# kngwyu/rogue-gym

Measured on AMD Instinct MI355X. Metric: env-steps/sec (whole node) at 65 536 envs, 32x16 mini-dungeon, higher is better.
Workload: dtype u8/u16 integer state, f32 observation; 1 GPU; config-mini.json 32x16, 65536 envs per GPU (65536 total), gray-image obs [N,1,16,32] f32, max_steps 1000, auto-reset; envs_per_gpu=65536, parallelism=env-sharded x1, no data-path collective

## Files before the change

### rogue-gym_amd/csrc/rg_api.cpp

```cpp
#include <hip/hip_runtime.h>
#include <dlfcn.h>

#include <algorithm>
#include <cstdio>
#include <cstdlib>
#include <cstring>
#include <mutex>
#include <random>
#include <string>
#include <vector>

#include "../../include/rogue_gym_hip.h"
#include "rg_state.h"
#include "rg_state_io.h"
#include "rg_action_mask.h"
#include "rg_path.h"
#include "rg_route.h"
#include "rg_episode.h"
#include "rg_monsters.h"

extern "C" {
typedef struct ncclComm *ncclComm_t;
typedef struct { char internal[128]; } ncclUniqueId;
typedef int ncclResult_t;
// ... 11 lines not shown
void rgk_export(const RgState *S, uint32_t *err_any, void *o_screen, void *o_hist, void *o_status, void *o_flags, uint32_t *o_err, hipStream_t st);
int rgk_regen_lanes_supported(const RgConfig *c, int maze_cap);
int rgk_step_bound_capable(const RgConfig *c);
int rgk_regen_lanes(const RgState *SP, const RgConfig *c, uint32_t *q, int32_t *list, int bulk, int waves, int slots, hipStream_t st, hipEvent_t ev0, hipEvent_t ev1);
void rgk_debug_descend(const RgState *S, const RgConfig *c, hipStream_t st);
void rgk_render(const RgState *S, const RgConfig *c, hipStream_t st);
void rgk_encode(const uint8_t *screen, const uint8_t *hist, const int32_t *status, uint32_t *flags, uint32_t *err_any, int n, int hw, size_t rs, size_t rst,
                int symbols, int planes_sym, uint32_t sflag, int with_hist, int kind, float *out, const int32_t *ext, hipStream_t st);
void rgk_pack(const RgState *S, int with_hist, uint8_t *out, hipStream_t st);
void rgk_scatter_rows(const void *src, void *dst, const int32_t *ext, int n, int row_bytes, hipStream_t st);
void rgk_gather_keys(const uint8_t *keys, const int32_t *ext, uint8_t *dst, int n, hipStream_t st);
int rgk_obs(const RgState *S, const RgConfig *c, uint32_t sflag, int with_hist, int kind, float *out, uint32_t *err_any, int planes_sym, int bound, hipStream_t st, hipEvent_t ev0, hipEvent_t ev1);
int rgk_redraw(const RgState *S, const RgConfig *c, hipStream_t st);
int rgk_obs_tail_capable(const RgState *S, const RgConfig *c);
int rgk_step_tail_capable(const RgConfig *c);
void rgk_obs_resid(const RgState *S, const RgConfig *c, float *out, hipStream_t st, hipEvent_t ev0, hipEvent_t ev1);
int rgk_obs_typed(const RgState *S, const RgConfig *c, int kind, int dtype, uint32_t sflag, int with_hist, int planes_sym, void *out, uint32_t *err_any, hipStream_t st, hipEvent_t ev0,
                  hipEvent_t ev1);
int rgk_obs_crop(const RgState *S, const RgConfig *c, int kind, int ry, int rx, uint32_t sflag, int with_hist, int planes_sym, float *out, int32_t *centers,
                 uint32_t *err_any, hipStream_t st);
int rgk_crop_typed(const RgState *S, const RgConfig *c, int kind, int dtype, int ry, int rx, uint32_t sflag, int with_hist, int planes_sym, void *out, int32_t *centers,
                   uint32_t *err_any, hipStream_t st, hipEvent_t ev0, hipEvent_t ev1);
void rgk_action_mask(const RgState *S, const RgConfig *c, const uint8_t *keys, int n_keys, uint8_t *mask, uint8_t *sample, uint64_t seed, uint64_t draw, hipStream_t st,
                     hipEvent_t ev0, hipEvent_t ev1);
void rgk_path(const RgState *S, const RgConfig *c, uint32_t goals, const int32_t *gcell, uint16_t *field, int32_t *dist, uint8_t *key, hipStream_t st);
void rgk_route(const RgState *S, const RgConfig *c, uint32_t goals, uint32_t fallback, uint32_t mode, const int32_t *gcell, int32_t *dist, uint8_t *key, uint8_t *tier,
               hipStream_t st);
void rgk_episode(const RgState *S, const RgConfig *c, const RgEpisode *A, int slots, const int32_t *ids, const uint8_t *mask, int cut, int record, uint32_t serial,
                 hipStream_t st);
void rgk_monsters(const RgState *S, const RgConfig *c, uint32_t mode, int cap, int16_t *table, int32_t *threat, hipStream_t st);
void rgk_state_save(const RgState *S, const RgIoLayout *L, const uint64_t *desc, const uint32_t *guard, const int32_t *ids, int k, uint8_t *out, hipStream_t st);
void rgk_state_load(const RgState *S, const RgIoLayout *L, const uint64_t *desc, const uint32_t *guard, const int32_t *ids, int k, const uint8_t *recs, uint32_t rec_bytes, uint8_t *ok,
                    uint8_t *mark, hipStream_t st);
void rgk_state_stairs(const RgState *S, const RgIoLayout *L, uint8_t *mark, hipStream_t st);
void rgk_reset_compact(const uint8_t *mask, int n, int32_t *list, uint32_t *cnt, hipStream_t st);
void rgk_build_list(const RgState *S, const RgConfig *c, const int32_t *list, const uint32_t *cnt, uint8_t *mark, hipStream_t st);
}

#define RG_ENC_CUT_TICKS 4000u
#define RG_TIMED_KERNELS 5
struct rg_handle {
    RgParsed parsed;
    RgConfig cfg;
    RgState S;
    RgState SP;
    bool spares = false;
    uint32_t *lane_q = nullptr; int32_t *lane_list = nullptr;
    hipStream_t side3 = nullptr;
    hipStream_t side2 = nullptr;
    int lane_flip = 0;
    uint64_t lane_last = 0;
    uint8_t *pin_keys = nullptr;
    uint32_t *pin_err = nullptr;
    bool lane_regen = false;
    uint64_t step_count = 0;
    hipStream_t side = nullptr;
    int regen_idle_after = -1;
    int regen_bulk = 0;
    int device = 0;
    hipStream_t stream = nullptr;
    std::vector<void *> allocs;
    uint32_t *d_err = nullptr;
    uint8_t *d_keys = nullptr;
    bool render_pending = false;
    float *bound_out = nullptr; int bound_kind = 0; bool bound_valid = false;
    int32_t *obs_list_mem = nullptr; uint32_t *obs_cnt_mem = nullptr; float *gray_lut_mem = nullptr;
    bool tail_enc = false, tail_enc_off = false;
    int bound_steps = 0;
    int stair_gen = 0;
    float *obs_scratch = nullptr;
    size_t obs_scratch_cap = 0;
    std::vector<uint64_t> seed_lo, seed_hi;
    std::vector<uint8_t> reseed;
    std::vector<uint64_t> range_lo, range_span;
    unsigned long long *d_probe = nullptr;
    std::vector<rg_handle *> sub;
    std::vector<int> g_of, l_of;
    int32_t *d_ext = nullptr;
    std::vector<int32_t> ext;
    uint8_t *d_keys_sub = nullptr;
    int planes_sym = 0;
    bool screens_stale = true;
// ... 160 lines not shown
              dev_alloc(h, &S.dlevel, n) && dev_alloc(h, &S.steps, n) && dev_alloc(h, &S.flags, n) && dev_alloc(h, &S.reward, n) && dev_alloc(h, &S.done, n) &&
              dev_alloc(h, &S.rng, 12 * n) && dev_alloc(h, &S.seed_lo, n) && dev_alloc(h, &S.seed_hi, n) && dev_alloc(h, &S.reseed, n) &&
              dev_alloc(h, &S.room_rect, nr * n) && dev_alloc(h, &S.room_meta, nr * n) &&
              dev_alloc(h, &S.mon_w0, nr * n) && dev_alloc(h, &S.mon_hp, nr * n) && dev_alloc(h, &S.mon_exp, nr * n) &&
              dev_alloc(h, &S.mon_cnt, n) && dev_alloc(h, &S.gold_pos, nr * n) && dev_alloc(h, &S.gold_amt, nr * n) &&
              dev_alloc(h, &S.edge_a, ne * n) && dev_alloc(h, &S.edge_b, ne * n) &&
              dev_alloc(h, &S.maze_stack, (size_t)maze_cap * n) && dev_alloc(h, &S.build_ctr, n) && dev_alloc(h, &S.stats, RG_STAT_COLS * h->stat_rows) && dev_alloc(h, &S.stair_list, 2 * n) && dev_alloc(h, &S.stair_cnt, 8) && dev_alloc(h, &S.stair_mark, 2 * n) &&
              dev_alloc(h, &S.dc_map, h->cfg.n_enemies > 0 ? n * RG_DIST_SLOTS * hw : 16) && dev_alloc(h, &S.dc_key, RG_DIST_SLOTS * n) &&
              dev_alloc(h, &S.dc_head, n) && dev_alloc(h, &S.dc_len, n) && dev_alloc(h, &S.dc_part, n) && dev_alloc(h, &S.dc_own, n) && dev_alloc(h, &S.status, n * 10) &&
              dev_alloc(h, &h->d_err, 4) && dev_alloc(h, &h->d_keys, n);
    if (ok && nr <= RG_OBS_MAX_ROOMS) ok = dev_alloc(h, &S.obs_rec, n * (size_t)RG_OBS_REC_WORDS(nr));
    if (ok && nr <= RG_OVL_MAX && getenv("ROGUE_GYM_HIP_NO_MIRROR_UPDATE") == nullptr)
        ok = dev_alloc(h, &S.ovl, (nr + 1) * n) && hipMemset(S.ovl, 0xff, (nr + 1) * n * 2) == hipSuccess;
    {
        if (ok && rgk_step_tail_capable(&h->cfg) && S.ovl && S.obs_rec) {
            ok = dev_alloc(h, &S.enc_stamp, n) && ensure_gray_lut(h) == 0;
            h->tail_enc = ok;
            S.enc_cut = RG_ENC_CUT_TICKS;
            if (const char *ev = RG_DEV_ENV("ROGUE_GYM_HIP_ENC_CUT")) S.enc_cut = (uint32_t)atoi(ev);
        }
    }
    h->spares = auto_reset != 0 && getenv("ROGUE_GYM_HIP_NO_SPARES") == nullptr;
    h->lane_regen = h->spares && getenv("ROGUE_GYM_HIP_WAVE_REGEN") == nullptr && rgk_regen_lanes_supported(&h->cfg, maze_cap) > 0;
    const char *slots_env = getenv("ROGUE_GYM_HIP_SP_SLOTS");
    S.sp_slots = h->lane_regen ? (slots_env ? atoi(slots_env) : 4) : 1;
    if (S.sp_slots < 1 || S.sp_slots > 8) S.sp_slots = 4;
    const size_t ns = n * (size_t)S.sp_slots;
    ok = ok && dev_alloc(h, &S.sp_ready, ns) && dev_alloc(h, &h->d_probe, 4) && dev_alloc(h, &S.launch_mark, 4);
    if (ok && h->cfg.n_enemies > 0 && RG_PARTIAL_MAPS(h->cfg.width, h->cfg.height, (int)nr))
        ok = dev_alloc(h, &S.dc_walk, n * RG_DIST_SLOTS * h->cfg.height * RG_WALK_WORDS(h->cfg.width));
    S.full_bfs = getenv("ROGUE_GYM_HIP_FULL_BFS") != nullptr;
    S.keep_spares = getenv("ROGUE_GYM_HIP_KEEP_SPARES") != nullptr;
    S.err_any = h->d_err;
    if (ok && !h->range_lo.empty()) {
// ... 251 lines not shown
    }
    h->S.stair_gen = h->stair_gen++;
    { TimedLaunch t(h, 3); rgk_build(&h->S, &h->cfg, h->stream); }
    HIPCHK(h, hipGetLastError());
    h->render_pending = true;
    h->bound_valid = false;
    return 0;
}

static int obs_common(rg_t *h, uint32_t status_flag, int with_hist, int kind, float *out_dev);
int rg_step(rg_t *h, const uint8_t *keys, int keys_on_device) { return rg_step_prefix(h, keys, h->S.n, keys_on_device); }
int rg_step_obs_gray(rg_t *h, const uint8_t *keys, int keys_on_device, uint32_t status_flag, int with_hist, float *out_dev) {
    const bool enc = h->tail_enc && !h->tail_enc_off && h->sub.empty() && (status_flag & 0x1ffu) == 0 && !with_hist && !h->bound_out && out_dev && rgk_obs_tail_capable(&h->S, &h->cfg);
    if (enc) {
        h->S.enc_out = out_dev;
        h->S.enc_step = (uint32_t)(h->step_count % 0xffffffffull) + 1u;
    }
    const int rc = rg_step_prefix(h, keys, h->S.n, keys_on_device);
    h->S.enc_out = nullptr;
    if (rc) return 1;
    if (!enc) return obs_common(h, status_flag, with_hist, 0, out_dev);
    {
        TimedLaunch t(h, 2, true);
        rgk_obs_resid(&h->S, &h->cfg, out_dev, h->stream, t.start_ev(), t.stop_ev());
    }
    HIPCHK(h, hipGetLastError());
    h->render_pending = false;
    h->bound_valid = false;
    h->bound_steps = 0;
    return 0;
}

int rg_step_prefix(rg_t *h, const uint8_t *keys, int n_keys, int keys_on_device) {
    HIPCHK(h, hipSetDevice(h->device));
// ... 1491 lines not shown
```

### rogue-gym_amd/csrc/rg_kernels.hip

```cpp


#include "rg_device.h"


#include "rg_gen.h"


#ifdef RG_FINE_PROF
#define PFM(id) pf.mark(id)
#else
#define PFM(id) ((void)0)
#endif
struct Prof {
    unsigned long long *p; unsigned long long t, t0, r0; int k;
    __device__ __forceinline__ void start(unsigned long long *pp) { p = pp ? pp + (size_t)blockIdx.x * 64 : nullptr; k = 0; if (p) { r0 = __builtin_amdgcn_s_memrealtime(); t = t0 = __builtin_amdgcn_s_memtime(); } }
    __device__ __forceinline__ void rec(int phase, unsigned long long v) {
        if (p && threadIdx.x == 0 && k < 61) p[1 + k++] = ((unsigned long long)phase << 48) | (v & 0xffffffffffffull);
    }
    __device__ __forceinline__ void mark(int phase) {
        if (!p) return;
        unsigned long long now = __builtin_amdgcn_s_memtime();
        rec(phase, now - t);
        t = now;
    }
// ... 2036 lines not shown
    }
    if (did_hit) react |= R_STATUS;
    return false;
}

__device__ __forceinline__ uint32_t base_glyph(const RgConfig &c, uint32_t v, int y) {
    const bool inner = y >= 1 && y < c.height - 1;
    uint32_t gl = ' ';
    if (inner && (v & C_VISIBLE)) gl = glyph_of(v);
    if (inner && (v & (C_VISIBLE | C_DRAWN))) gl = ((v & C_GOLD) ? (uint32_t)'*' : gl) | 0x80u;
    return gl;
}
#define OVL_SHOW 0x80u
#define OVL_UNKNOWN 0x40u
#define OVL_NONE 0xffffu
template <bool BND>
__device__ __forceinline__ bool mirror_update(const RgState &S, const RgConfig &c, const Env &E, const Win &w, uint32_t react, int rid0) {
    const int W = c.width, nrooms = c.room_num_x * c.room_num_y, n = E.n;
    int e = E.e;
    asm volatile("" : "+v"(e));
    uint8_t *scr = S.screen + (size_t)e * S.hw;
    float *og = (BND && S.bound_gray) ? S.bound_gray + (size_t)e * S.hw : nullptr;
    const __attribute__((address_space(3))) float *lutg = (const __attribute__((address_space(3))) float *)(g_smem + STEP_LDS_LUT);
    auto put = [&](int idx, uint32_t g) {
        scr[idx] = (uint8_t)g;
        if constexpr (BND) { if (og) og[idx] = lutg[g & 0x7fu]; }
    };
    int ln = threadIdx.x;
    asm volatile("" : "+v"(ln));
    const lds_u32 *mc = (const lds_u32 *)(g_smem + STEP_LDS_MC) + ln;
    const lds_u32 *ovl_l = (const lds_u32 *)(g_smem + STEP_LDS_OVL) + ln;
    const uint32_t ds = ovl_l[0] & 0x1ffffffu;
    const int px = E.px, py = E.py, rid = room_id_of(c, px, py);
    auto in_win = [&](int x, int y) { const int i = x - w.ox, j = y - w.oy; return i >= -2 && i <= 2 && j >= -2 && j <= 2; };
    auto dirty_at = [&](int x, int y) { return in_win(x, y) && ((ds >> WIN_K(x - w.ox, y - w.oy)) & 1u); };
    const int rsel = rid == rid0 ? 0 : 2;
    const uint32_t r_rect = ovl_l[(RG_OVL_MAX + 2 + rsel) * WAVE], r_meta = ovl_l[(RG_OVL_MAX + 3 + rsel) * WAVE] & 0xffu;
    const __attribute__((address_space(3))) uint8_t *mt = (const __attribute__((address_space(3))) uint8_t *)(ovl_l - ln + (RG_OVL_MAX + 6) * WAVE);
    uint32_t actp = 0;
    bool far = false;
// ... 135 lines not shown
                if (s0 + k < nrooms) {
                    const size_t g = (size_t)(s0 + k) * n + e;
                    S.room_rect[g] = rr[k]; S.room_meta[g] = rm[k]; S.mon_w0[g] = mw[k]; S.mon_hp[g] = mh[k]; S.mon_exp[g] = me[k]; S.gold_pos[g] = gp[k]; S.gold_amt[g] = ga[k];
                    if (S.obs_rec) {
                        uint32_t *rec = S.obs_rec + (size_t)e * RG_OBS_REC_WORDS(nrooms);
                        rec[s0 + k] = mw[k]; rec[nrooms + 1 + s0 + k] = rr[k]; reinterpret_cast<uint8_t *>(&rec[2 * nrooms + 1])[s0 + k] = rm[k];
                    }
                    if (S.ovl) S.ovl[(size_t)(s0 + k) * n + e] = (uint16_t)(((mw[k] >> 24) & MF_ALIVE) ? ((mw[k] & 0xffffu) | 0x40u) : 0xffffu);
                }
        }
    }
    __syncthreads();
    if (taken && !(S.keep_spares && S.reseed[e] == 0)) __hip_atomic_store(&S.sp_ready[es], 0u, __ATOMIC_RELAXED, __HIP_MEMORY_SCOPE_AGENT);
}

#ifndef ENC_BATCH
#define ENC_BATCH 8
#endif
__device__ __forceinline__ void tail_encode(const RgState &S, const int lane, const int e, const bool encl) {
    typedef float f4v __attribute__((ext_vector_type(4)));
    const uint64_t em = __ballot(encl);
    if (encl) S.enc_stamp[e] = S.enc_step;
    if (!em) return;
    const int ebase = __builtin_amdgcn_readfirstlane(e - lane);
    asm volatile("s_waitcnt vmcnt(0)" ::: "memory");
    const __attribute__((address_space(3))) float *lut = (const __attribute__((address_space(3))) float *)(g_smem + STEP_LDS_LUT);
    const uint32_t *mir = reinterpret_cast<const uint32_t *>(S.screen) + lane;
    f4v *img = reinterpret_cast<f4v *>(S.enc_out) + lane;
    uint64_t rem = em;
    int last = 0;
    struct Batch { int env[ENC_BATCH]; uint32_t w0[ENC_BATCH], w1[ENC_BATCH]; };
    auto load = [&](Batch &b) {
#pragma unroll
        for (int k = 0; k < ENC_BATCH; k++) {
            last = rem ? __builtin_ctzll(rem) : last;
            rem &= rem - (rem ? 1ull : 0ull);
            b.env[k] = ebase + last;
            const uint32_t *m = mir + (size_t)b.env[k] * 128;
            b.w0[k] = __hip_atomic_load(m, __ATOMIC_RELAXED, __HIP_MEMORY_SCOPE_AGENT);
            b.w1[k] = __hip_atomic_load(m + WAVE, __ATOMIC_RELAXED, __HIP_MEMORY_SCOPE_AGENT);
        }
    };
    auto gray4 = [&](uint32_t w) {
        w &= 0x7f7f7f7fu;
        f4v v = {lut[w & 0xff], lut[(w >> 8) & 0xff], lut[(w >> 16) & 0xff], lut[w >> 24]};
        return v;
    };
    auto store = [&](const Batch &b) {
#pragma unroll
        for (int k = 0; k < ENC_BATCH; k++) {
            f4v *o = img + (size_t)b.env[k] * 128;
            __builtin_nontemporal_store(gray4(b.w0[k]), o);
            __builtin_nontemporal_store(gray4(b.w1[k]), o + WAVE);
        }
    };
    const int nb = (__popcll(em) + ENC_BATCH - 1) / ENC_BATCH;
    Batch cur, nxt;
    load(cur);
    load(nxt);
    store(cur);
#pragma nounroll
    for (int b = 1; b < nb; b++) {
        cur = nxt;
        load(nxt);
        store(cur);
    }
}

template <int BW, int GM, bool BND = false, bool ENC = false>
__device__ __forceinline__ void step_wave(const RgState &S, const RgState *__restrict__ SPd, const RgConfig &c, const uint8_t *__restrict__ keys, int use_spares, int stage_off,
                                          const int e, const bool valid_in, const int stair_role) {
    uint16_t *lds_grid = reinterpret_cast<uint16_t *>(g_smem + stage_off);
    const int lane = threadIdx.x;
    Prof pf; pf.start(S.prof);
    const unsigned long long enc_t0 = ENC ? __builtin_amdgcn_s_memrealtime() : 0ull;
    Env E;
    E.err = 0; E.on_stairs = 0;
    uint32_t react = 0, err = 0, old_flags = 0, steps = 0, flags = 0;
    int act = ACT_NOOP, dir = 0;
    int gold0 = 0;
    bool live = false;
    bool ui_dead = false, terminal = false;
    bool inc_done = false;
    bool taken = false;
    uint32_t n_bfs = 0, n_inline = 0, n_taken = 0, n_cont = 0;
    uint32_t key = 0, nxs = RG_NX_NONE;
    bool listed = false;
    const int nrooms_k = c.room_num_x * c.room_num_y;
    E.mc = (lds_u32 *)(g_smem + STEP_LDS_MC) + lane;
    const uint32_t glyph_r = S.ovl ? c.mon[lane & 31].tile : 0u;
    if (valid_in) {
        listed = S.stair_mark[(size_t)(S.stair_gen & 1) * S.n + e] != 0;
        uint32_t nxk = 0;
        if (S.nx_state) {
            nxs = __hip_atomic_load(&S.nx_state[e], __ATOMIC_RELAXED, __HIP_MEMORY_SCOPE_AGENT);
            nxk = __hip_atomic_load(&S.nx_rng[(size_t)3 * S.n + e], __ATOMIC_RELAXED, __HIP_MEMORY_SCOPE_AGENT);
        }
        old_flags = S.flags[e];
// ... 19 lines not shown
            act = decode_key(key, dir);
            if (act == ACT_INVALID) err = RG_FLAG_ERR_KEY;
            else {
                klog_push(S, e, key);
                if (old_flags & RG_FLAG_DEAD) err = RG_FLAG_ERR_DEAD;
                else live = true;
            }
        }
    }
    pf.mark(0);
    bool need_gen = false, descends = false;
    Win w;
    w.v = (lds_u16 *)(g_smem + STEP_LDS_WIN) + lane;
    lds_u32 *ovl_l = (lds_u32 *)(g_smem + STEP_LDS_OVL) + lane;
    ovl_l[0] = 0;
    if ((BND && S.bound_gray) || ENC) {
        typedef const __attribute__((address_space(1))) void *gptr;
        typedef __attribute__((address_space(3))) void *lptr;
        __builtin_amdgcn_global_load_lds((gptr)(S.gray_lut + lane), (lptr)(g_smem + STEP_LDS_LUT), 4, 0, 0);
        __builtin_amdgcn_global_load_lds((gptr)(S.gray_lut + 64 + lane), (lptr)(g_smem + STEP_LDS_LUT + 256), 4, 0, 0);
    }
    if (S.ovl && lane < RG_MAX_ENEMY_KINDS + 6)
        ((__attribute__((address_space(3))) uint8_t *)(g_smem + STEP_LDS_OVL + (RG_OVL_MAX + 6) * WAVE * 4))[lane] = (uint8_t)glyph_r;
    if (S.ovl) {
        typedef const __attribute__((address_space(1))) void *gptr;
        typedef __attribute__((address_space(3))) void *lptr;
        lds_u32 *base = (lds_u32 *)(g_smem + STEP_LDS_OVL);
        const size_t es = valid_in ? (size_t)e : 0;
#pragma unroll
        for (int s0 = 0; s0 <= RG_OVL_MAX; s0++)
            __builtin_amdgcn_global_load_lds((gptr)(S.ovl + (size_t)(s0 <= nrooms_k ? s0 : 0) * S.n + es), (lptr)(base + (1 + s0) * WAVE), 2, 0, 0);
// ... 138 lines not shown
            if (running) win_load(c, E.cell, w, E.px, E.py);
        }
        if (live) {
            flags = (react & 0x7f00u);
            if (react & R_REDRAW) flags |= RG_FLAG_REDRAW | ((react & R_HIST_STALE) ? RG_FLAG_HIST_STALE : 0);
            else flags |= old_flags & (RG_FLAG_REDRAW | RG_FLAG_HIST_STALE);
            flags |= old_flags & (RG_FLAG_HIST_LAG | RG_FLAG_HIST_DIRTY | (BND ? RG_FLAG_SCR_CHANGED : 0u));
            if ((react & R_HIST_CHANGED) || descends) flags |= RG_FLAG_HIST_DIRTY;
            if (react & R_STATUS) write_status(S, c, E);
            if (ui_dead) flags |= RG_FLAG_DEAD;
            steps += 1;
            terminal = (react & R_GRAVE) || steps >= c.max_steps;
            need_gen = terminal && c.auto_reset;
            if (S.ovl && (react & R_REDRAW) && !descends && !need_gen && act != ACT_MOVE_UNTIL &&
                !(old_flags & (RG_FLAG_REDRAW | RG_FLAG_HIST_STALE | RG_FLAG_HIST_LAG | RG_FLAG_HIST_DIRTY)) && !(ovl_l[0] >> 31)) {
                if (mirror_update<BND>(S, c, E, w, react, room_id_of(c, w.ox, w.oy))) flags = (flags & ~(RG_FLAG_REDRAW | RG_FLAG_HIST_DIRTY)) | ((!BND || S.bound_gray) ? 0u : RG_FLAG_SCR_CHANGED);
                inc_done = true;
            }
        }
    }
    pf.mark(6);
    int et = e;
    asm volatile("" : "+v"(et));
    E.e = et;
    bool pend = false; uint64_t pm = 0; uint32_t lbase = 0;
    bool encl = false;
    if (BND && S.obs_list) {
        const uint32_t fw = (live ? ((terminal && c.auto_reset) ? RG_FLAG_REDRAW : flags) : old_flags);
        pend = valid && (fw & (RG_FLAG_REDRAW | RG_FLAG_SCR_CHANGED));
        pm = __ballot(pend);
        if (pm && lane == 0) lbase = atomicAdd(&S.obs_cnt[S.obs_par], (uint32_t)__popcll(pm));
    }
    if (S.stats) {
        const uint32_t cnt[8] = {(uint32_t)__popcll(__ballot(live && terminal && c.auto_reset)), (uint32_t)__popcll(__ballot(descends)),
                                 wave_sum(n_bfs), wave_sum(n_inline), wave_sum(n_taken), (uint32_t)__popcll(__ballot(live && (react & R_REDRAW))),
                                 (uint32_t)__popcll(__ballot(live)), (BW == 1 || BW == 2) ? wave_sum(n_cont) : 0u};
        const uint32_t n_nx = (uint32_t)__popcll(__ballot(descends && nxs == RG_NX_HIT));
        int ln = threadIdx.x;
        asm volatile("" : "+v"(ln));
        if (ln < RG_STAT_COLS) {
            uint32_t mine = ln == 8 ? n_nx : 0u;
// ... 13 lines not shown
        if (terminal && c.auto_reset) {
            if (taken) {
                E.dlevel = 1; E.gold = c.init_gold; E.hp = E.hpmax = c.init_hp; E.plvl = 1; E.exp = 0; E.food = c.hunger_time;
            }
            write_status(S, c, E);
            S.dc_len[et] = 0; S.dc_head[et] = 0; S.dc_part[et] = 0; S.dc_own[et] = 0;
            steps = 0;
            flags = RG_FLAG_REDRAW | RG_FLAG_HIST_DIRTY;
            klog_new_episode(S, et);
        }
        if (E.err) { flags |= E.err; atomicOr(S.err_any, E.err); }
        if (terminal) flags |= RG_FLAG_TERMINAL;
        if (!taken) store_env(S, E);
        S.steps[et] = steps;
        S.flags[et] = flags;
        if (ENC) encl = !(flags & RG_FLAG_REDRAW);
        S.done[et] = terminal ? 1 : 0;
        if (S.ovl && !taken && !inc_done && ((react & R_REDRAW) || descends || (terminal && c.auto_reset))) {
            for (int s0 = 0; s0 < nrooms_k; s0++) {
                const uint32_t mw = E.mc[s0 * WAVE];
                S.ovl[(size_t)s0 * S.n + et] = (uint16_t)(((mw >> 24) & MF_ALIVE) ? ((mw & 0xffffu) | OVL_UNKNOWN) : OVL_NONE);
            }
            S.ovl[(size_t)nrooms_k * S.n + et] = (uint16_t)(POS(E.px, E.py) | OVL_UNKNOWN);
        }
        if (S.obs_rec && (flags & RG_FLAG_REDRAW) && !taken) {
            uint32_t *rec = S.obs_rec + (size_t)et * RG_OBS_REC_WORDS(nrooms_k);
            for (int s0 = 0; s0 < nrooms_k; s0 += 4) {
                uint32_t m4[4];
#pragma unroll
                for (int k = 0; k < 4; k++) m4[k] = E.mc[(s0 + k < nrooms_k ? s0 + k : s0) * WAVE];
                if (s0 + 4 <= nrooms_k) *reinterpret_cast<uint4 *>(rec + s0) = make_uint4(m4[0], m4[1], m4[2], m4[3]);
// ... 22 lines not shown
                st_pub<true>(&q[0], E.rd.x); st_pub<true>(&q[n], E.rd.y); st_pub<true>(&q[2 * n], E.rd.z); st_pub<true>(&q[3 * n], E.rd.w);
                st_pub<true>(&q[8 * n], E.ri.x); st_pub<true>(&q[9 * n], E.ri.y); st_pub<true>(&q[10 * n], E.ri.z); st_pub<true>(&q[11 * n], E.ri.w);
                st_pub<true>(&S.nx->level[et], E.dlevel);
            }
            asm volatile("s_waitcnt vmcnt(0)" ::: "memory");
            if (ask) __hip_atomic_store(&S.nx_state[et], RG_NX_ASKED, __ATOMIC_RELAXED, __HIP_MEMORY_SCOPE_AGENT);
        }
    }
    if (BND && pm) {
        const uint32_t lb = uni(lbase);
        if (pend) S.obs_list[(size_t)S.obs_par * S.n + lb + lanes_below(pm)] = et;
    }
    take_spares(S, SPd, c, lane, et, taken, on_next);
    stair_publish(S, lane, et, valid, on_next);
    pf.mark(7);
    if constexpr (ENC) {
        const bool late = __builtin_amdgcn_s_memrealtime() - enc_t0 > (unsigned long long)S.enc_cut;
        tail_encode(S, lane, et, encl && !late);
        pf.mark(31);
    }
    pf.finish();
}

#define STAIR_BLOCKS 256

#define RG_STEP_BLOCK_BODY(BWV, GMV, BNDV, ENCV) \
    __builtin_amdgcn_s_setprio(3); \
    const int lane = threadIdx.x; \
    if (blockIdx.x == 0 && lane == 0) { \
        stair_recycle(S); \
        if (BNDV && S.obs_cnt) S.obs_cnt[S.obs_par ^ 1] = 0;   \
        __hip_atomic_store(S.launch_mark, (uint32_t)S.stair_gen + 1u, __ATOMIC_RELAXED, __HIP_MEMORY_SCOPE_AGENT);   \
    } \
    const bool stair = parity >= 0 && (int)blockIdx.x < STAIR_BLOCKS; \
    const int32_t *list = S.stair_list + (size_t)(S.stair_gen & 1) * S.n; \
// ... 7 lines not shown
        if (!stair || __any(v)) step_wave<BWV, GMV, BNDV, ENCV>(S, SPd, c, keys, use_spares, stage_off, e, v, parity >= 0 ? (stair ? 1 : 2) : 0); \
        if (!stair || items <= STAIR_BLOCKS) break; \
        __syncthreads(); \
        uint32_t t = 0; \
        if (lane == 0) t = atomicAdd(next, 1u); \
        i0 = STAIR_BLOCKS + (int)uni(t); \
    }
template <int BW, bool BND = false>
__global__ void __launch_bounds__(WAVE) k_step(RgState S, const RgState *__restrict__ SPd, RgConfig c, const uint8_t *__restrict__ keys, int use_spares, int stage_off, int epw,
                                               int parity) {
    RG_STEP_BLOCK_BODY(BW, (BW != 0 ? 1 : 0), BND, false)
}
template <bool BND, bool ENC = false>
__global__ void __launch_bounds__(WAVE) __attribute__((amdgpu_waves_per_eu(2, 2)))
k_step_w32(RgState S, const RgState *__restrict__ SPd, RgConfig c, const uint8_t *__restrict__ keys, int use_spares, int stage_off, int epw, int parity) {
    RG_STEP_BLOCK_BODY(0, 0, BND, ENC)
}
__global__ void __launch_bounds__(WAVE) k_step_huge(RgState S, const RgState *__restrict__ SPd, RgConfig c, const uint8_t *__restrict__ keys, int use_spares, int stage_off,
                                                    int epw, int parity) {
    RG_STEP_BLOCK_BODY(4, 2, false, false)
}
#undef RG_STEP_BLOCK_BODY

static int gen_mode_of(const RgConfig *c) { const int nr = c->room_num_x * c->room_num_y; return nr <= 32 ? 0 : (nr <= 64 ? 1 : 2); }
extern "C" {
void rgk_build(const RgState *S, const RgConfig *c, hipStream_t st) {
    int hw = c->width * c->height;
    size_t smem = GEN_SLOT_BYTES(hw, c->room_num_x * c->room_num_y);
    const dim3 grid((S->n + BUILD_EPB - 1) / BUILD_EPB);
    switch (gen_mode_of(c)) {
// ... 31 lines not shown
    const size_t bfs_hi = n32 ? 0 : (size_t)10 * ((c->width + 63) / 64) * WAVE * 8;
    if (bfs_hi > stage) stage = bfs_hi;
    stage = (stage + 15) & ~(size_t)15;
    const int stage_off = STEP_LDS_MC + c->room_num_x * c->room_num_y * WAVE * 4;
    if (stage_off_out) *stage_off_out = stage_off;
    return (size_t)stage_off + stage;
}
size_t rgk_step_lds_per_cu(const RgConfig *c) { return step_lds(c, nullptr) * ((c->width <= 32 && gen_mode_of(c) == 0) ? 8 : 4); }
int rgk_step_bound_capable(const RgConfig *c) {
    const int hw = c->width * c->height;
    if (gen_mode_of(c) == 2) return 0;
    if (c->width <= 32 && gen_mode_of(c) == 0) return 1;
    return (c->width <= 96 && hw <= 4096 && c->width > 64) ? 1 : 0;
}
int rgk_step_tail_capable(const RgConfig *c) { return (c->width <= 32 && gen_mode_of(c) == 0 && c->width * c->height == 512) ? 1 : 0; }
int rgk_step(const RgState *S, const RgState *SP_dev, const RgConfig *c, const uint8_t *keys, int use_spares, int parity, hipStream_t st, hipEvent_t ev0, hipEvent_t ev1) {
    const bool bnd = S->obs_list != nullptr && rgk_step_bound_capable(c);
    int hw = c->width * c->height;
    const bool n32 = c->width <= 96 && hw <= 4096;
    int stage_off = 0;
    const size_t smem = step_lds(c, &stage_off);
    const int epw = rgk_step_epw(S->n, (c->width <= 32 && gen_mode_of(c) == 0) ? 2 : 1);
    const int nb = (S->n + epw - 1) / epw;
    const dim3 grid(parity >= 0 ? STAIR_BLOCKS + nb : nb), block(WAVE);
#define RG_LAUNCH_STEP(K) do { if (ev0 || ev1) hipExtLaunchKernelGGL(K, grid, block, (uint32_t)smem, st, ev0, ev1, 0, *S, SP_dev, *c, keys, use_spares, stage_off, epw, parity); \
                               else hipLaunchKernelGGL(K, grid, block, smem, st, *S, SP_dev, *c, keys, use_spares, stage_off, epw, parity); } while (0)
    if (gen_mode_of(c) == 2) {
        static size_t raised[64] = {0};
        int dev = 0;
        (void)hipGetDevice(&dev);
        if (dev < 0 || dev >= 64 || smem > raised[dev]) {
            if (hipFuncSetAttribute(reinterpret_cast<const void *>(k_step_huge), hipFuncAttributeMaxDynamicSharedMemorySize, (int)smem) == hipSuccess && dev >= 0 && dev < 64) raised[dev] = smem;
        }
        RG_LAUNCH_STEP(k_step_huge);
    } else if (c->width <= 32 && gen_mode_of(c) == 0) { if (bnd) RG_LAUNCH_STEP(k_step_w32<true>); else if (S->enc_out) RG_LAUNCH_STEP((k_step_w32<false, true>)); else RG_LAUNCH_STEP(k_step_w32<false>); }
    else if (n32 && c->width <= 64) RG_LAUNCH_STEP(k_step<1>);
    else if (n32) { if (bnd) RG_LAUNCH_STEP((k_step<2, true>)); else RG_LAUNCH_STEP(k_step<2>); }
    else if (c->width <= 128) RG_LAUNCH_STEP(k_step<3>);
    else RG_LAUNCH_STEP(k_step<4>);
// ... 38 lines not shown
```

### rogue-gym_amd/csrc/rg_obs.hip

```cpp
#include <cstdlib>
#include "rg_device.h"

#define RENDER_THREADS 256
__device__ __forceinline__ bool in_same_room(const RgState &S, const RgConfig &c, int e, int ax, int ay, int bx, int by) {
    int id = room_id_of(c, ax, ay);
    if (id < 0 || room_id_of(c, bx, by) != id) return false;
    uint8_t meta = S.room_meta[id * S.n + e];
    if ((meta & RM_KIND_MASK) == RK_EMPTY) return true;
    int x0, y0, x1, y1;
    unpack_rect(S.room_rect[id * S.n + e], x0, y0, x1, y1);
    bool ina = ax >= x0 && ax < x1 && ay >= y0 && ay < y1, inb = bx >= x0 && bx < x1 && by >= y0 && by < y1;
    return ina == inb;
}

__global__ void __launch_bounds__(RENDER_THREADS) k_render(RgState S, RgConfig c) {
    __shared__ uint8_t s_scr[RG_MAX_W * RG_MAX_H];
    const int tid = threadIdx.x, W = c.width, H = c.height, HW = W * H, n = S.n;
    const int nrooms = c.room_num_x * c.room_num_y;
    for (int e = blockIdx.x; e < n; e += gridDim.x) {
        const uint32_t fl = S.flags[e];
        if (!(fl & RG_FLAG_REDRAW)) continue;
        const uint16_t *cell = S.cell + (size_t)e * HW;
        const bool upd_hist = !(fl & RG_FLAG_HIST_STALE);
        uint8_t *hist = S.hist + (size_t)e * HW;
// ... 469 lines not shown

#ifndef OBS_RESID_RUN
#define OBS_RESID_RUN 4
#endif
#ifndef OBS_RESID_WAVES
#define OBS_RESID_WAVES 16384
#endif
__global__ void __launch_bounds__(WAVE) k_obs_resid(RgState S, RgConfig c, float *__restrict__ out) {
    __shared__ float lutf[128];
    __shared__ uint8_t mtile[RG_MAX_ENEMY_KINDS + 6];
    __shared__ __align__(16) uint8_t scr[512];
    __shared__ ObsTabs tb;
    const int lane = threadIdx.x, W = c.width, HW = W * c.height, Q4 = HW >> 2, Q8 = HW >> 3, n = S.n;
    const int nrooms = c.room_num_x * c.room_num_y, rec_words = RG_OBS_REC_WORDS(nrooms);
    const int nruns = (n + OBS_RESID_RUN - 1) / OBS_RESID_RUN;
    auto load_run = [&](int r, uint32_t &fl, uint32_t &stamp) {
        const int base = r * OBS_RESID_RUN;
        const bool in = r < nruns && lane < OBS_RESID_RUN && base + lane < n;
        fl = in ? S.flags[base + lane] : 0u;
        stamp = in ? S.enc_stamp[base + lane] : S.enc_step;
    };
    uint32_t fl_cur, st_cur;
    load_run(blockIdx.x, fl_cur, st_cur);
    lutf[lane] = S.gray_lut[lane];
    lutf[lane + WAVE] = S.gray_lut[lane + WAVE];
    for (int g = lane; g < RG_MAX_ENEMY_KINDS + 6; g += WAVE) mtile[g] = c.mon[g].tile;
    lds_barrier();
    auto gray4 = [&](uint32_t w) {
        w &= 0x7f7f7f7fu;
        float4 v; v.x = lutf[w & 0xff]; v.y = lutf[(w >> 8) & 0xff]; v.z = lutf[(w >> 16) & 0xff]; v.w = lutf[w >> 24];
        return v;
    };
    auto load_tiles = [&](int e, uint4 &v, uint32_t &rec) {
        v = lane < Q8 ? reinterpret_cast<const uint4 *>(S.cell + (size_t)e * HW)[lane] : make_uint4(0, 0, 0, 0);
        rec = lane < rec_words ? S.obs_rec[(size_t)e * rec_words + lane] : 0u;
    };
    for (int r = blockIdx.x; r < nruns; r += gridDim.x) {
        const int base = r * OBS_RESID_RUN;
        const uint32_t fl = fl_cur;
        const bool need = st_cur != S.enc_step;
        load_run(r + gridDim.x, fl_cur, st_cur);
        uint64_t rmask = __ballot(need && (fl & RG_FLAG_REDRAW));
        const uint64_t smask = __ballot(need && !(fl & RG_FLAG_REDRAW));
        if (!(rmask | smask)) continue;
        uint4 tv = make_uint4(0, 0, 0, 0);
        uint32_t trec = 0;
        if (rmask) load_tiles(base + __builtin_ctzll(rmask), tv, trec);
        const uint32_t *m = reinterpret_cast<const uint32_t *>(S.screen) + (size_t)base * Q4;
        float4 *o = reinterpret_cast<float4 *>(out) + (size_t)base * Q4;
        uint32_t w0[OBS_RESID_RUN], w1[OBS_RESID_RUN];
#pragma unroll
        for (int i = 0; i < OBS_RESID_RUN; i++) {
            w0[i] = w1[i] = 0u;
            if ((smask >> i) & 1) { w0[i] = m[i * Q4 + lane]; w1[i] = m[i * Q4 + lane + WAVE]; }
        }
#pragma unroll
        for (int i = 0; i < OBS_RESID_RUN; i++) {
            if (!((smask >> i) & 1)) continue;
            store_obs(&o[i * Q4 + lane], gray4(w0[i]));
            store_obs(&o[i * Q4 + lane + WAVE], gray4(w1[i]));
        }
        while (rmask) {
            const int i = __builtin_ctzll(rmask);
            rmask &= rmask - 1;
            const int e = base + i;
            const uint32_t fle = __builtin_amdgcn_readlane(fl, i);
            const uint4 v = tv;
            const uint32_t t_rec = trec;
            if (rmask) load_tiles(base + __builtin_ctzll(rmask), tv, trec);
            RG_OBS_REDRAW_ENV();
        }
    }
}

#define RG_PUBLIC_FLAGS (RG_FLAG_TERMINAL | RG_FLAG_DEAD | RG_FLAG_MSG_MASK | RG_FLAG_ERR_MASK)
// ... 575 lines not shown
```

### rogue-gym_amd/csrc/rg_state.h

```cpp
#pragma once
#include <cstdint>

#include "rg_config.h"

#define C_SURF_MASK 0x0007u
#define C_DOOR      0x0008u
#define C_ATTR_SHIFT 4
#define C_VISITED   0x0010u
#define C_HIDDEN    0x0020u
#define C_VISIBLE   0x0040u
#define C_DRAWN     0x0080u
#define C_LOCKED    0x0100u
#define C_DARK      0x0200u
#define C_ATTR_MASK 0x03f0u
#define C_MAZE      0x0400u
#define C_GOLD      0x0800u

enum { S_PASSAGE = 0, S_FLOOR, S_WALLX, S_WALLY, S_STAIR, S_DOOR, S_TRAP, S_NONE };

#define RM_KIND_MASK 0x03u
#define RM_DARK      0x04u
#define RM_VISITED   0x08u
#define RM_HAS_GOLD  0x10u
enum { RK_NORMAL = 0, RK_MAZE = 1, RK_EMPTY = 2 };
// ... 56 lines not shown
    uint16_t *dc_key;
    uint8_t *dc_head, *dc_len;
    uint16_t *dc_part, *dc_own;
    uint32_t *dc_walk;
    int keep_spares;
    int full_bfs;
    unsigned long long *prof;
    uint32_t *sp_ready;
    int32_t sp_slots;
    int32_t *status;
    uint32_t *obs_rec;
    uint16_t *ovl;
    float *bound_gray;
    const float *gray_lut;
    float *enc_out;
    uint32_t *enc_stamp;
    uint32_t enc_step;
    uint32_t enc_cut;
    int32_t *obs_list;
    uint32_t *obs_cnt;
    int32_t obs_par;
    uint8_t *klog;
    uint32_t *klog_len;
    uint8_t *klog_cur;
    int32_t klog_cap;
    unsigned long long *stats;
    uint8_t *stair_mark;
    int32_t *stair_list;
    uint32_t *stair_cnt;
    int32_t stair_gen;
    uint32_t *launch_mark;
    uint8_t *on_stairs;
    uint32_t *nx_state;
// ... 8 lines not shown
```

Baseline: 828.9 million env-steps/s.

## Move tail encoding into dedicated helper blocks and track dirty rows for residual

Drops the per-wave tail encode that ran at the end of each step block under a time cutoff. Extra low-priority helper blocks are appended to the step grid; they sleep for a fixed delay and then convert all mirrored screens to gray floats, overlapping with the step work. The step kernel now records a 16-bit mask of which screen rows changed during incremental mirror updates, so the residual obs pass rewrites only dirty rows rather than whole screens. The helpers may read screens before the step blocks finish writing them, which is why the residual pass redoes every changed row. They also take CU slots away from the step blocks and re-encode every env each step.

Measured after the change: 860.0 million env-steps/s, median of 6. 3.8% higher.

```diff
diff --git a/rogue-gym_amd/csrc/rg_api.cpp b/rogue-gym_amd/csrc/rg_api.cpp
--- a/rogue-gym_amd/csrc/rg_api.cpp
+++ b/rogue-gym_amd/csrc/rg_api.cpp
@@ -49,6 +49,7 @@
 int rgk_redraw(const RgState *S, const RgConfig *c, hipStream_t st);
 int rgk_obs_tail_capable(const RgState *S, const RgConfig *c);
 int rgk_step_tail_capable(const RgConfig *c);
+int rgk_step_enc_helpers(int n, int want);
 void rgk_obs_resid(const RgState *S, const RgConfig *c, float *out, hipStream_t st, hipEvent_t ev0, hipEvent_t ev1);
 int rgk_obs_typed(const RgState *S, const RgConfig *c, int kind, int dtype, uint32_t sflag, int with_hist, int planes_sym, void *out, uint32_t *err_any, hipStream_t st, hipEvent_t ev0,
                   hipEvent_t ev1);
@@ -72,7 +73,7 @@
 void rgk_build_list(const RgState *S, const RgConfig *c, const int32_t *list, const uint32_t *cnt, uint8_t *mark, hipStream_t st);
 }
 
-#define RG_ENC_CUT_TICKS 4000u
+#define RG_ENC_DELAY_TICKS 2500u
 #define RG_TIMED_KERNELS 5
 struct rg_handle {
     RgParsed parsed;
@@ -101,6 +102,7 @@
     float *bound_out = nullptr; int bound_kind = 0; bool bound_valid = false;
     int32_t *obs_list_mem = nullptr; uint32_t *obs_cnt_mem = nullptr; float *gray_lut_mem = nullptr;
     bool tail_enc = false, tail_enc_off = false;
+    int enc_helpers = 0;
     int bound_steps = 0;
     int stair_gen = 0;
     float *obs_scratch = nullptr;
@@ -291,10 +293,12 @@
         ok = dev_alloc(h, &S.ovl, (nr + 1) * n) && hipMemset(S.ovl, 0xff, (nr + 1) * n * 2) == hipSuccess;
     {
         if (ok && rgk_step_tail_capable(&h->cfg) && S.ovl && S.obs_rec) {
-            ok = dev_alloc(h, &S.enc_stamp, n) && ensure_gray_lut(h) == 0;
+            ok = dev_alloc(h, &S.enc_rows, n) && ensure_gray_lut(h) == 0;
             h->tail_enc = ok;
-            S.enc_cut = RG_ENC_CUT_TICKS;
-            if (const char *ev = RG_DEV_ENV("ROGUE_GYM_HIP_ENC_CUT")) S.enc_cut = (uint32_t)atoi(ev);
+            const char *hv = RG_DEV_ENV("ROGUE_GYM_HIP_ENC_HELPERS"), *dv = RG_DEV_ENV("ROGUE_GYM_HIP_ENC_DELAY"), *cv = RG_DEV_ENV("ROGUE_GYM_HIP_ENC_CUT");
+            h->enc_helpers = rgk_step_enc_helpers((int)n, hv ? atoi(hv) : 0);
+            if (cv && atoi(cv) == 0) h->enc_helpers = 0;
+            S.enc_delay = dv ? (uint32_t)atoi(dv) : RG_ENC_DELAY_TICKS;
         }
     }
     h->spares = auto_reset != 0 && getenv("ROGUE_GYM_HIP_NO_SPARES") == nullptr;
@@ -576,10 +580,11 @@
     const bool enc = h->tail_enc && !h->tail_enc_off && h->sub.empty() && (status_flag & 0x1ffu) == 0 && !with_hist && !h->bound_out && out_dev && rgk_obs_tail_capable(&h->S, &h->cfg);
     if (enc) {
         h->S.enc_out = out_dev;
-        h->S.enc_step = (uint32_t)(h->step_count % 0xffffffffull) + 1u;
+        h->S.enc_helpers = h->enc_helpers;
     }
     const int rc = rg_step_prefix(h, keys, h->S.n, keys_on_device);
     h->S.enc_out = nullptr;
+    h->S.enc_helpers = 0;
     if (rc) return 1;
     if (!enc) return obs_common(h, status_flag, with_hist, 0, out_dev);
     {
diff --git a/rogue-gym_amd/csrc/rg_kernels.hip b/rogue-gym_amd/csrc/rg_kernels.hip
--- a/rogue-gym_amd/csrc/rg_kernels.hip
+++ b/rogue-gym_amd/csrc/rg_kernels.hip
@@ -2074,8 +2074,8 @@
 #define OVL_SHOW 0x80u
 #define OVL_UNKNOWN 0x40u
 #define OVL_NONE 0xffffu
-template <bool BND>
-__device__ __forceinline__ bool mirror_update(const RgState &S, const RgConfig &c, const Env &E, const Win &w, uint32_t react, int rid0) {
+template <bool BND, bool ENC = false>
+__device__ __forceinline__ bool mirror_update(const RgState &S, const RgConfig &c, const Env &E, const Win &w, uint32_t react, int rid0, uint32_t &rows) {
     const int W = c.width, nrooms = c.room_num_x * c.room_num_y, n = E.n;
     int e = E.e;
     asm volatile("" : "+v"(e));
@@ -2084,6 +2084,7 @@
     const __attribute__((address_space(3))) float *lutg = (const __attribute__((address_space(3))) float *)(g_smem + STEP_LDS_LUT);
     auto put = [&](int idx, uint32_t g) {
         scr[idx] = (uint8_t)g;
+        if constexpr (ENC) rows |= 1u << (idx >> 5);
         if constexpr (BND) { if (og) og[idx] = lutg[g & 0x7fu]; }
     };
     int ln = threadIdx.x;
@@ -2249,31 +2250,36 @@
     if (taken && !(S.keep_spares && S.reseed[e] == 0)) __hip_atomic_store(&S.sp_ready[es], 0u, __ATOMIC_RELAXED, __HIP_MEMORY_SCOPE_AGENT);
 }
 
-#ifndef ENC_BATCH
-#define ENC_BATCH 8
+#ifndef ENC_RUN
+#define ENC_RUN 4
 #endif
-__device__ __forceinline__ void tail_encode(const RgState &S, const int lane, const int e, const bool encl) {
+#define ENC_DELAY_MAX 20000u
+__device__ __forceinline__ void enc_helper(const RgState &S, const int hb, const int nh) {
     typedef float f4v __attribute__((ext_vector_type(4)));
-    const uint64_t em = __ballot(encl);
-    if (encl) S.enc_stamp[e] = S.enc_step;
-    if (!em) return;
-    const int ebase = __builtin_amdgcn_readfirstlane(e - lane);
-    asm volatile("s_waitcnt vmcnt(0)" ::: "memory");
+    __builtin_amdgcn_s_setprio(0);
+    const int lane = threadIdx.x;
+    const int n = S.n, nruns = (n + ENC_RUN - 1) / ENC_RUN;
+    if (hb >= nruns) return;
+    lds_u32 *lutw = (lds_u32 *)(g_smem + STEP_LDS_LUT);
+    lutw[lane] = __float_as_uint(S.gray_lut[lane]);
+    lutw[lane + WAVE] = __float_as_uint(S.gray_lut[lane + WAVE]);
+    __syncthreads();
+    if (S.enc_delay) {
+        const unsigned long long t0 = __builtin_amdgcn_s_memrealtime(), lim = S.enc_delay < ENC_DELAY_MAX ? S.enc_delay : ENC_DELAY_MAX;
+        while (__builtin_amdgcn_s_memrealtime() - t0 < lim) __builtin_amdgcn_s_sleep(16);
+    }
     const __attribute__((address_space(3))) float *lut = (const __attribute__((address_space(3))) float *)(g_smem + STEP_LDS_LUT);
     const uint32_t *mir = reinterpret_cast<const uint32_t *>(S.screen) + lane;
     f4v *img = reinterpret_cast<f4v *>(S.enc_out) + lane;
-    uint64_t rem = em;
-    int last = 0;
-    struct Batch { int env[ENC_BATCH]; uint32_t w0[ENC_BATCH], w1[ENC_BATCH]; };
-    auto load = [&](Batch &b) {
-#pragma unroll
-        for (int k = 0; k < ENC_BATCH; k++) {
-            last = rem ? __builtin_ctzll(rem) : last;
-            rem &= rem - (rem ? 1ull : 0ull);
-            b.env[k] = ebase + last;
-            const uint32_t *m = mir + (size_t)b.env[k] * 128;
-            b.w0[k] = __hip_atomic_load(m, __ATOMIC_RELAXED, __HIP_MEMORY_SCOPE_AGENT);
-            b.w1[k] = __hip_atomic_load(m + WAVE, __ATOMIC_RELAXED, __HIP_MEMORY_SCOPE_AGENT);
+    struct Run { uint32_t w0[ENC_RUN], w1[ENC_RUN]; };
+    auto load = [&](int r, Run &R) {
+#pragma unroll
+        for (int k = 0; k < ENC_RUN; k++) {
+            int e = r * ENC_RUN + k;
+            e = e < n ? e : n - 1;
+            const uint32_t *m = mir + (size_t)e * 128;
+            R.w0[k] = __hip_atomic_load(m, __ATOMIC_RELAXED, __HIP_MEMORY_SCOPE_AGENT);
+            R.w1[k] = __hip_atomic_load(m + WAVE, __ATOMIC_RELAXED, __HIP_MEMORY_SCOPE_AGENT);
         }
     };
     auto gray4 = [&](uint32_t w) {
@@ -2281,24 +2287,26 @@
         f4v v = {lut[w & 0xff], lut[(w >> 8) & 0xff], lut[(w >> 16) & 0xff], lut[w >> 24]};
         return v;
     };
-    auto store = [&](const Batch &b) {
-#pragma unroll
-        for (int k = 0; k < ENC_BATCH; k++) {
-            f4v *o = img + (size_t)b.env[k] * 128;
-            __builtin_nontemporal_store(gray4(b.w0[k]), o);
-            __builtin_nontemporal_store(gray4(b.w1[k]), o + WAVE);
+    auto store = [&](int r, const Run &R) {
+#pragma unroll
+        for (int k = 0; k < ENC_RUN; k++) {
+            int e = r * ENC_RUN + k;
+            e = e < n ? e : n - 1;
+            f4v *o = img + (size_t)e * 128;
+            __builtin_nontemporal_store(gray4(R.w0[k]), o);
+            __builtin_nontemporal_store(gray4(R.w1[k]), o + WAVE);
         }
     };
-    const int nb = (__popcll(em) + ENC_BATCH - 1) / ENC_BATCH;
-    Batch cur, nxt;
-    load(cur);
-    load(nxt);
-    store(cur);
+    Run cur, nxt;
+    int r = hb;
+    load(r, cur);
+    load(r + nh, nxt);
+    store(r, cur);
 #pragma nounroll
-    for (int b = 1; b < nb; b++) {
+    for (r += nh; r < nruns; r += nh) {
         cur = nxt;
-        load(nxt);
-        store(cur);
+        load(r + nh, nxt);
+        store(r, cur);
     }
 }
 
@@ -2308,7 +2316,6 @@
     uint16_t *lds_grid = reinterpret_cast<uint16_t *>(g_smem + stage_off);
     const int lane = threadIdx.x;
     Prof pf; pf.start(S.prof);
-    const unsigned long long enc_t0 = ENC ? __builtin_amdgcn_s_memrealtime() : 0ull;
     Env E;
     E.err = 0; E.on_stairs = 0;
     uint32_t react = 0, err = 0, old_flags = 0, steps = 0, flags = 0;
@@ -2317,6 +2324,7 @@
     bool live = false;
     bool ui_dead = false, terminal = false;
     bool inc_done = false;
+    uint32_t enc_rows = 0;
     bool taken = false;
     uint32_t n_bfs = 0, n_inline = 0, n_taken = 0, n_cont = 0;
     uint32_t key = 0, nxs = RG_NX_NONE;
@@ -2366,7 +2374,7 @@
     w.v = (lds_u16 *)(g_smem + STEP_LDS_WIN) + lane;
     lds_u32 *ovl_l = (lds_u32 *)(g_smem + STEP_LDS_OVL) + lane;
     ovl_l[0] = 0;
-    if ((BND && S.bound_gray) || ENC) {
+    if (BND && S.bound_gray) {
         typedef const __attribute__((address_space(1))) void *gptr;
         typedef __attribute__((address_space(3))) void *lptr;
         __builtin_amdgcn_global_load_lds((gptr)(S.gray_lut + lane), (lptr)(g_smem + STEP_LDS_LUT), 4, 0, 0);
@@ -2535,7 +2543,7 @@
             need_gen = terminal && c.auto_reset;
             if (S.ovl && (react & R_REDRAW) && !descends && !need_gen && act != ACT_MOVE_UNTIL &&
                 !(old_flags & (RG_FLAG_REDRAW | RG_FLAG_HIST_STALE | RG_FLAG_HIST_LAG | RG_FLAG_HIST_DIRTY)) && !(ovl_l[0] >> 31)) {
-                if (mirror_update<BND>(S, c, E, w, react, room_id_of(c, w.ox, w.oy))) flags = (flags & ~(RG_FLAG_REDRAW | RG_FLAG_HIST_DIRTY)) | ((!BND || S.bound_gray) ? 0u : RG_FLAG_SCR_CHANGED);
+                if (mirror_update<BND, ENC>(S, c, E, w, react, room_id_of(c, w.ox, w.oy), enc_rows)) flags = (flags & ~(RG_FLAG_REDRAW | RG_FLAG_HIST_DIRTY)) | ((!BND || S.bound_gray) ? 0u : RG_FLAG_SCR_CHANGED);
                 inc_done = true;
             }
         }
@@ -2545,7 +2553,6 @@
     asm volatile("" : "+v"(et));
     E.e = et;
     bool pend = false; uint64_t pm = 0; uint32_t lbase = 0;
-    bool encl = false;
     if (BND && S.obs_list) {
         const uint32_t fw = (live ? ((terminal && c.auto_reset) ? RG_FLAG_REDRAW : flags) : old_flags);
         pend = valid && (fw & (RG_FLAG_REDRAW | RG_FLAG_SCR_CHANGED));
@@ -2589,7 +2596,6 @@
         if (!taken) store_env(S, E);
         S.steps[et] = steps;
         S.flags[et] = flags;
-        if (ENC) encl = !(flags & RG_FLAG_REDRAW);
         S.done[et] = terminal ? 1 : 0;
         if (S.ovl && !taken && !inc_done && ((react & R_REDRAW) || descends || (terminal && c.auto_reset))) {
             for (int s0 = 0; s0 < nrooms_k; s0++) {
@@ -2642,11 +2648,7 @@
     take_spares(S, SPd, c, lane, et, taken, on_next);
     stair_publish(S, lane, et, valid, on_next);
     pf.mark(7);
-    if constexpr (ENC) {
-        const bool late = __builtin_amdgcn_s_memrealtime() - enc_t0 > (unsigned long long)S.enc_cut;
-        tail_encode(S, lane, et, encl && !late);
-        pf.mark(31);
-    }
+    if constexpr (ENC) { if (valid) S.enc_rows[et] = (uint16_t)(S.enc_helpers ? enc_rows : 0xffffu); }
     pf.finish();
 }
 
@@ -2684,6 +2686,10 @@
 template <bool BND, bool ENC = false>
 __global__ void __launch_bounds__(WAVE) __attribute__((amdgpu_waves_per_eu(2, 2)))
 k_step_w32(RgState S, const RgState *__restrict__ SPd, RgConfig c, const uint8_t *__restrict__ keys, int use_spares, int stage_off, int epw, int parity) {
+    if constexpr (ENC) {
+        const int first_helper = (int)gridDim.x - S.enc_helpers;
+        if ((int)blockIdx.x >= first_helper) { enc_helper(S, (int)blockIdx.x - first_helper, S.enc_helpers); return; }
+    }
     RG_STEP_BLOCK_BODY(0, 0, BND, ENC)
 }
 __global__ void __launch_bounds__(WAVE) k_step_huge(RgState S, const RgState *__restrict__ SPd, RgConfig c, const uint8_t *__restrict__ keys, int use_spares, int stage_off,
@@ -2745,6 +2751,13 @@
     return (c->width <= 96 && hw <= 4096 && c->width > 64) ? 1 : 0;
 }
 int rgk_step_tail_capable(const RgConfig *c) { return (c->width <= 32 && gen_mode_of(c) == 0 && c->width * c->height == 512) ? 1 : 0; }
+#define ENC_HELPERS 384
+int rgk_step_enc_helpers(int n, int want) {
+    const int nruns = (n + ENC_RUN - 1) / ENC_RUN;
+    int h = ENC_HELPERS;
+    if (want > 0) h = want > 2048 ? 2048 : want;
+    return h < nruns ? h : nruns;
+}
 int rgk_step(const RgState *S, const RgState *SP_dev, const RgConfig *c, const uint8_t *keys, int use_spares, int parity, hipStream_t st, hipEvent_t ev0, hipEvent_t ev1) {
     const bool bnd = S->obs_list != nullptr && rgk_step_bound_capable(c);
     int hw = c->width * c->height;
@@ -2753,7 +2766,8 @@
     const size_t smem = step_lds(c, &stage_off);
     const int epw = rgk_step_epw(S->n, (c->width <= 32 && gen_mode_of(c) == 0) ? 2 : 1);
     const int nb = (S->n + epw - 1) / epw;
-    const dim3 grid(parity >= 0 ? STAIR_BLOCKS + nb : nb), block(WAVE);
+    const bool enc = !bnd && S->enc_out && c->width <= 32 && gen_mode_of(c) == 0;
+    const dim3 grid((parity >= 0 ? STAIR_BLOCKS + nb : nb) + (enc ? S->enc_helpers : 0)), block(WAVE);
 #define RG_LAUNCH_STEP(K) do { if (ev0 || ev1) hipExtLaunchKernelGGL(K, grid, block, (uint32_t)smem, st, ev0, ev1, 0, *S, SP_dev, *c, keys, use_spares, stage_off, epw, parity); \
                                else hipLaunchKernelGGL(K, grid, block, smem, st, *S, SP_dev, *c, keys, use_spares, stage_off, epw, parity); } while (0)
     if (gen_mode_of(c) == 2) {
diff --git a/rogue-gym_amd/csrc/rg_obs.hip b/rogue-gym_amd/csrc/rg_obs.hip
--- a/rogue-gym_amd/csrc/rg_obs.hip
+++ b/rogue-gym_amd/csrc/rg_obs.hip
@@ -507,14 +507,14 @@
     const int lane = threadIdx.x, W = c.width, HW = W * c.height, Q4 = HW >> 2, Q8 = HW >> 3, n = S.n;
     const int nrooms = c.room_num_x * c.room_num_y, rec_words = RG_OBS_REC_WORDS(nrooms);
     const int nruns = (n + OBS_RESID_RUN - 1) / OBS_RESID_RUN;
-    auto load_run = [&](int r, uint32_t &fl, uint32_t &stamp) {
+    auto load_run = [&](int r, uint32_t &fl, uint32_t &rows) {
         const int base = r * OBS_RESID_RUN;
         const bool in = r < nruns && lane < OBS_RESID_RUN && base + lane < n;
         fl = in ? S.flags[base + lane] : 0u;
-        stamp = in ? S.enc_stamp[base + lane] : S.enc_step;
-    };
-    uint32_t fl_cur, st_cur;
-    load_run(blockIdx.x, fl_cur, st_cur);
+        rows = in ? (uint32_t)S.enc_rows[base + lane] : 0u;
+    };
+    uint32_t fl_cur, rw_cur;
+    load_run(blockIdx.x, fl_cur, rw_cur);
     lutf[lane] = S.gray_lut[lane];
     lutf[lane + WAVE] = S.gray_lut[lane + WAVE];
     for (int g = lane; g < RG_MAX_ENEMY_KINDS + 6; g += WAVE) mtile[g] = c.mon[g].tile;
@@ -528,13 +528,13 @@
         v = lane < Q8 ? reinterpret_cast<const uint4 *>(S.cell + (size_t)e * HW)[lane] : make_uint4(0, 0, 0, 0);
         rec = lane < rec_words ? S.obs_rec[(size_t)e * rec_words + lane] : 0u;
     };
+    const int band = lane >> 3;
     for (int r = blockIdx.x; r < nruns; r += gridDim.x) {
         const int base = r * OBS_RESID_RUN;
-        const uint32_t fl = fl_cur;
-        const bool need = st_cur != S.enc_step;
-        load_run(r + gridDim.x, fl_cur, st_cur);
-        uint64_t rmask = __ballot(need && (fl & RG_FLAG_REDRAW));
-        const uint64_t smask = __ballot(need && !(fl & RG_FLAG_REDRAW));
+        const uint32_t fl = fl_cur, rows = rw_cur;
+        load_run(r + gridDim.x, fl_cur, rw_cur);
+        uint64_t rmask = __ballot(fl & RG_FLAG_REDRAW);
+        const uint64_t smask = __ballot(!(fl & RG_FLAG_REDRAW) && rows != 0u);
         if (!(rmask | smask)) continue;
         uint4 tv = make_uint4(0, 0, 0, 0);
         uint32_t trec = 0;
@@ -545,13 +545,18 @@
 #pragma unroll
         for (int i = 0; i < OBS_RESID_RUN; i++) {
             w0[i] = w1[i] = 0u;
-            if ((smask >> i) & 1) { w0[i] = m[i * Q4 + lane]; w1[i] = m[i * Q4 + lane + WAVE]; }
+            if ((smask >> i) & 1) {
+                const uint32_t ri = __builtin_amdgcn_readlane(rows, i);
+                if ((ri >> band) & 1u) w0[i] = m[i * Q4 + lane];
+                if ((ri >> (8 + band)) & 1u) w1[i] = m[i * Q4 + lane + WAVE];
+            }
         }
 #pragma unroll
         for (int i = 0; i < OBS_RESID_RUN; i++) {
             if (!((smask >> i) & 1)) continue;
-            store_obs(&o[i * Q4 + lane], gray4(w0[i]));
-            store_obs(&o[i * Q4 + lane + WAVE], gray4(w1[i]));
+            const uint32_t ri = __builtin_amdgcn_readlane(rows, i);
+            if ((ri >> band) & 1u) store_obs(&o[i * Q4 + lane], gray4(w0[i]));
+            if ((ri >> (8 + band)) & 1u) store_obs(&o[i * Q4 + lane + WAVE], gray4(w1[i]));
         }
         while (rmask) {
             const int i = __builtin_ctzll(rmask);
diff --git a/rogue-gym_amd/csrc/rg_state.h b/rogue-gym_amd/csrc/rg_state.h
--- a/rogue-gym_amd/csrc/rg_state.h
+++ b/rogue-gym_amd/csrc/rg_state.h
@@ -94,9 +94,9 @@
     float *bound_gray;
     const float *gray_lut;
     float *enc_out;
-    uint32_t *enc_stamp;
-    uint32_t enc_step;
-    uint32_t enc_cut;
+    uint16_t *enc_rows;
+    int32_t enc_helpers;
+    uint32_t enc_delay;
     int32_t *obs_list;
     uint32_t *obs_cnt;
     int32_t obs_par;
```
